# AiRyunn/BoT

Measured on NVIDIA B200. Metric: GAT layer fwd+bwd edges/sec (ogbn-proteins shape), higher is better.
Workload: dtype f32

## Files before the change

bot_b200/csrc/common.cuh:

```cuda
#pragma once

#include <atomic>
#include <cuda_runtime.h>
#include <stdint.h>
#include <stdio.h>

#include <type_traits>

#include "botgat.h"

namespace botgat {

void set_error(const char* fmt, ...);
const char* env_str(const char* name);
int64_t env_int(const char* name, int64_t dflt);
extern std::atomic<long long> g_launches;
#define BG_LAUNCHED(n) (::botgat::g_launches.fetch_add(n, std::memory_order_relaxed))

#define BG_CHECK(expr)                                                                  \
  do {                                                                                  \
    cudaError_t _e = (expr);                                                            \
    if (_e != cudaSuccess) {                                                            \
      ::botgat::set_error("%s:%d: %s -> %s", __FILE__, __LINE__, #expr, cudaGetErrorString(_e)); \
      return -2;                                                                        \
    }                                                                                   \
  } while (0)

#define BG_REQUIRE(cond, ...)            \
  do {                                   \
    if (!(cond)) {                       \
      ::botgat::set_error(__VA_ARGS__);  \
      return -1;                         \
    }                                    \
  } while (0)

struct DeviceGuard {
  int prev = -1;
  explicit DeviceGuard(int dev) {
    cudaGetDevice(&prev);
    if (dev != prev) cudaSetDevice(dev);
  }
  ~DeviceGuard() {
    int cur;
    cudaGetDevice(&cur);
    if (cur != prev && prev >= 0) cudaSetDevice(prev);
  }
};

template <typename K>
static inline int resident_grid(K kernel, int block_threads, int64_t blocks_of_work) {
  int dev = 0, sms = 148, per_sm = 1;
  cudaGetDevice(&dev);
  cudaDeviceGetAttribute(&sms, cudaDevAttrMultiProcessorCount, dev);
  if (cudaOccupancyMaxActiveBlocksPerMultiprocessor(&per_sm, kernel, block_threads, 0) != cudaSuccess || per_sm < 1) per_sm = 1;
  const int64_t resident = (int64_t)sms * per_sm;
  return (int)(blocks_of_work < 1 ? 1 : (blocks_of_work < resident ? blocks_of_work : resident));
}

}

struct botgat_graph {
  int device = 0;
  int sm_count = 148;
  int64_t n_src = 0, n_dst = 0, n_edges = 0;
  int64_t max_in_deg = 0, max_out_deg = 0;
  int has_zero_in_degree = 0;
  int32_t *in_indptr = nullptr, *in_indices = nullptr, *in_eid = nullptr;
  int32_t *out_indptr = nullptr, *out_indices = nullptr, *out_eid = nullptr;
  int32_t *in_deg = nullptr, *out_deg = nullptr;
  int in_eid_identity = 0;
  int32_t* out_tile_order = nullptr;
  int tiles_s = 1, tiles_d = 1;
  struct SegTable {
    int n_items = 0;
    int n_slots = 0;
    int n_split = 0;
    int32_t *row = nullptr, *beg = nullptr, *end = nullptr, *slot = nullptr;
    int32_t *split_rows = nullptr, *split_first = nullptr;
  } seg_in, seg_out;
};

namespace botgat {

#ifndef BG_WPB
#define BG_WPB 4
#endif
constexpr int kWarpsPerBlock = BG_WPB;
constexpr unsigned kFull = 0xffffffffu;

__device__ __forceinline__ float leaky_relu(float z, float slope) {
  return z > 0.f ? z : (z == -INFINITY ? -INFINITY : z * slope);
}

__device__ __forceinline__ float warp_max(float v) {
#pragma unroll
  for (int o = 16; o > 0; o >>= 1) v = fmaxf(v, __shfl_xor_sync(kFull, v, o));
  return v;
}
__device__ __forceinline__ float warp_sum(float v) {
#pragma unroll
  for (int o = 16; o > 0; o >>= 1) v += __shfl_xor_sync(kFull, v, o);
  return v;
}

__device__ __forceinline__ uint32_t philox_u32(uint64_t seed, uint32_t eid, uint32_t head) {
  uint32_t c0 = eid, c1 = head >> 2, c2 = 0x9E3779B9u, c3 = 0xBB67AE85u;
  uint32_t k0 = (uint32_t)seed, k1 = (uint32_t)(seed >> 32);
#pragma unroll
  for (int r = 0; r < 10; ++r) {
    uint32_t hi0 = __umulhi(0xD2511F53u, c0), lo0 = 0xD2511F53u * c0;
    uint32_t hi1 = __umulhi(0xCD9E8D57u, c2), lo1 = 0xCD9E8D57u * c2;
    uint32_t n0 = hi1 ^ c1 ^ k0, n1 = lo1, n2 = hi0 ^ c3 ^ k1, n3 = lo0;
    c0 = n0; c1 = n1; c2 = n2; c3 = n3;
    k0 += 0x9E3779B9u; k1 += 0xBB67AE85u;
  }
  uint32_t sel = head & 3u;
  return sel == 0 ? c0 : sel == 1 ? c1 : sel == 2 ? c2 : c3;
}
__device__ __forceinline__ float philox_dropout_mul(uint64_t seed, uint32_t eid, uint32_t head, float p, float inv_keep) {
  float u = (float)(philox_u32(seed, eid, head) >> 8) * (1.0f / 16777216.0f);
  return u >= p ? inv_keep : 0.f;
}

template <int VW> struct Vec;
// ... 119 lines not shown
```

bot_b200/csrc/edge_ops.cu:

```cuda
#include <cub/cub.cuh>
#include <thrust/iterator/counting_iterator.h>
#include <thrust/iterator/transform_iterator.h>

#include "common.cuh"

namespace botgat {

static int env_pf() {
  return (int)env_int("BOTGAT_PF", 0);
}

template <int PF> __device__ __forceinline__ float4 ld_rec4(const float* p) {
  float4 r;
  if constexpr (PF == 64)
    asm("ld.global.nc.L2::64B.v4.f32 {%0,%1,%2,%3}, [%4];" : "=f"(r.x), "=f"(r.y), "=f"(r.z), "=f"(r.w) : "l"(p));
  else if constexpr (PF == 128)
    asm("ld.global.nc.L2::128B.v4.f32 {%0,%1,%2,%3}, [%4];" : "=f"(r.x), "=f"(r.y), "=f"(r.z), "=f"(r.w) : "l"(p));
  else if constexpr (PF == 256)
    asm("ld.global.nc.L2::256B.v4.f32 {%0,%1,%2,%3}, [%4];" : "=f"(r.x), "=f"(r.y), "=f"(r.z), "=f"(r.w) : "l"(p));
  else
    r = __ldg(reinterpret_cast<const float4*>(p));
  return r;
}
template <int PF> __device__ __forceinline__ float2 ld_rec2(const float* p) {
// ... 9 lines not shown
  if constexpr (PF == 64) asm("ld.global.nc.L2::64B.f32 %0, [%1];" : "=f"(r) : "l"(p));
  else if constexpr (PF == 128) asm("ld.global.nc.L2::128B.f32 %0, [%1];" : "=f"(r) : "l"(p));
  else if constexpr (PF == 256) asm("ld.global.nc.L2::256B.f32 %0, [%1];" : "=f"(r) : "l"(p));
  else r = __ldg(p);
  return r;
}

constexpr int kHMax = 8;

template <int VEC, int PF> __device__ __forceinline__ void load_record(const float* rec, int H, float (&v)[kHMax]) {
  if constexpr (VEC == 4) {
#pragma unroll
    for (int q = 0; q < kHMax / 4; ++q) {
      if (q * 4 < H) {
        const float4 t = ld_rec4<PF>(rec + q * 4);
        v[q * 4] = t.x; v[q * 4 + 1] = t.y; v[q * 4 + 2] = t.z; v[q * 4 + 3] = t.w;
      }
    }
  } else if constexpr (VEC == 2) {
#pragma unroll
    for (int q = 0; q < kHMax / 2; ++q) {
      if (q * 2 < H) {
        const float2 t = ld_rec2<PF>(rec + q * 2);
        v[q * 2] = t.x; v[q * 2 + 1] = t.y;
      }
    }
  } else {
#pragma unroll
    for (int q = 0; q < kHMax; ++q)
      if (q < H) v[q] = ld_rec1<PF>(rec + q);
  }
}
template <int VEC> __device__ __forceinline__ void store_record(float* rec, int H, const float (&v)[kHMax]) {
  if constexpr (VEC == 4) {
#pragma unroll
    for (int q = 0; q < kHMax / 4; ++q)
      if (q * 4 < H) *reinterpret_cast<float4*>(rec + q * 4) = make_float4(v[q * 4], v[q * 4 + 1], v[q * 4 + 2], v[q * 4 + 3]);
  } else if constexpr (VEC == 2) {
#pragma unroll
    for (int q = 0; q < kHMax / 2; ++q)
      if (q * 2 < H) *reinterpret_cast<float2*>(rec + q * 2) = make_float2(v[q * 2], v[q * 2 + 1]);
  } else {
#pragma unroll
    for (int q = 0; q < kHMax; ++q)
      if (q < H) rec[q] = v[q];
  }
}

static int record_vec(const void* p, int64_t ld, int H) {
  auto fits = [&](int w) { return ld % w == 0 && ((uintptr_t)p % (4 * w)) == 0 && ((H + w - 1) / w) * w <= ld; };
  return fits(4) ? 4 : (fits(2) ? 2 : 1);
}

__global__ void k_pack_keep(int64_t n_edges, const uint8_t* __restrict__ keep, uint32_t* __restrict__ bits) {
  const int64_t n_round = (n_edges + 31) & ~(int64_t)31;
  for (int64_t e = blockIdx.x * (int64_t)blockDim.x + threadIdx.x; e < n_round; e += (int64_t)gridDim.x * blockDim.x) {
    const unsigned b = __ballot_sync(0xffffffffu, e < n_edges && __ldg(keep + e) != 0);
    if ((threadIdx.x & 31) == 0) bits[e >> 5] = b;
  }
}

struct KeptMap {
  const uint32_t* bits;
  const int32_t* base;
  __device__ __forceinline__ int64_t rank(int64_t x) const {
    return __ldg(base + (x >> 5)) + __popc(__ldg(bits + (x >> 5)) & ((1u << (x & 31)) - 1u));
  }
  __device__ __forceinline__ bool kept(int64_t p) const { return (__ldg(bits + (p >> 5)) >> (p & 31)) & 1u; }
};

template <int VEC, int PF>
__global__ void k_edge_stage(int64_t n_edges, int h0, int Hn, const int32_t* __restrict__ eid,
                             const int32_t* __restrict__ order,
                             const float* __restrict__ src, int64_t ld, const uint8_t* __restrict__ keep,
                             const uint32_t* __restrict__ keep_bits, float* __restrict__ dst,
                             const KeptMap km, const int32_t* __restrict__ indices,
                             int32_t* __restrict__ sub_indices, int32_t* __restrict__ sub_eid) {
  for (int64_t t = blockIdx.x * (int64_t)blockDim.x + threadIdx.x; t < n_edges; t += (int64_t)gridDim.x * blockDim.x) {
    const int64_t p = order ? __ldg(order + t) : t;
    int64_t q = p;
    if (km.bits) {
      if (!km.kept(p)) continue;
      q = km.rank(p);
    }
    const int64_t e = __ldg(eid + p);
    float v[kHMax];
#pragma unroll
    for (int c = 0; c < kHMax; ++c) v[c] = 0.f;
    if (src) load_record<VEC, PF>(src + e * ld + h0, Hn, v);
    const bool dropped = keep_bits ? !((__ldg(keep_bits + (e >> 5)) >> (e & 31)) & 1u) : (keep && !__ldg(keep + e));
#pragma unroll
    for (int c = 0; c < kHMax; ++c)
      if (c < Hn) dst[(int64_t)(h0 + c) * n_edges + q] = dropped ? -INFINITY : v[c];
    if (sub_indices) {
      sub_indices[q] = __ldg(indices + p);
      if (sub_eid) sub_eid[q] = (int32_t)e;
    }
  }
}

template <int VEC>
__global__ void k_edge_unstage(int64_t n_edges, int h0, int Hn, int Hw, const int32_t* __restrict__ eid,
                               const int32_t* __restrict__ order, const KeptMap km,
                               const float* __restrict__ gz, float* __restrict__ dst, int64_t ld) {
  for (int64_t t = blockIdx.x * (int64_t)blockDim.x + threadIdx.x; t < n_edges; t += (int64_t)gridDim.x * blockDim.x) {
    const int64_t p = order ? __ldg(order + t) : t;
    const int64_t e = __ldg(eid + p);
    int64_t q = p;
    bool kept = true;
    if (km.bits) {
      kept = km.kept(p);
      q = km.rank(p);
    }
    float v[kHMax];
#pragma unroll
    for (int c = 0; c < kHMax; ++c) v[c] = (c < Hn && kept) ? __ldg(gz + (int64_t)(h0 + c) * n_edges + q) : 0.f;
    store_record<VEC>(dst + e * ld + h0, Hw, v);
  }
}

__global__ void k_kept_bits(int64_t n_edges, int64_t n_words, const int32_t* __restrict__ eid, const uint8_t* __restrict__ keep,
                            const uint32_t* __restrict__ keep_bits, uint32_t* __restrict__ bits) {
  for (int64_t p = blockIdx.x * (int64_t)blockDim.x + threadIdx.x; p < n_words * 32; p += (int64_t)gridDim.x * blockDim.x) {
    bool k = false;
    if (p < n_edges) {
      const int64_t e = eid ? __ldg(eid + p) : p;
      k = keep_bits ? ((__ldg(keep_bits + (e >> 5)) >> (e & 31)) & 1u) : __ldg(keep + e) != 0;
    }
    const unsigned b = __ballot_sync(0xffffffffu, k);
    if ((threadIdx.x & 31) == 0) bits[p >> 5] = b;
  }
}

struct WordCount {
  const uint32_t* bits;
  __device__ int operator()(int64_t w) const { return __popc(__ldg(bits + w)); }
};

__global__ void k_subset_bounds(int n_rows, const int32_t* __restrict__ indptr, int n_seg, const int32_t* __restrict__ seg_beg,
                                const int32_t* __restrict__ seg_end, const KeptMap km,
                                int32_t* __restrict__ sub_indptr, int32_t* __restrict__ sub_beg, int32_t* __restrict__ sub_end) {
  const int n = max(n_rows + 1, n_seg);
  for (int i = blockIdx.x * blockDim.x + threadIdx.x; i < n; i += gridDim.x * blockDim.x) {
    if (i <= n_rows) sub_indptr[i] = (int32_t)km.rank(__ldg(indptr + i));
    if (i < n_seg) {
      sub_beg[i] = (int32_t)km.rank(__ldg(seg_beg + i));
      sub_end[i] = (int32_t)km.rank(__ldg(seg_end + i));
    }
  }
}

template <int VEC, int PF>
__global__ void __launch_bounds__(256)
k_edge_reduce_dst(int n_items, int H, int h0, int Hn, const int32_t* __restrict__ indptr, const int32_t* __restrict__ eid,
                  const int32_t* __restrict__ seg_row, const int32_t* __restrict__ seg_beg,
                  const int32_t* __restrict__ seg_end, const int32_t* __restrict__ seg_slot,
                  const float* __restrict__ grad_ee, int64_t ld, float* __restrict__ grad_er, float* __restrict__ scratch) {
  const int warp = threadIdx.x >> 5, lane = threadIdx.x & 31;
  const int item = blockIdx.x * 8 + warp;
  if (item >= n_items) return;
  const int v = seg_row ? seg_row[item] : item;
  const int beg = seg_row ? seg_beg[item] : indptr[v], end = seg_row ? seg_end[item] : indptr[v + 1];
  const int slot = seg_row ? seg_slot[item] : -1;
  float s[kHMax];
#pragma unroll
  for (int q = 0; q < kHMax; ++q) s[q] = 0.f;
  for (int pos = beg + lane; pos < end; pos += 32) {
    float r[kHMax];
#pragma unroll
    for (int q = 0; q < kHMax; ++q) r[q] = 0.f;
    load_record<VEC, PF>(grad_ee + (int64_t)__ldg(eid + pos) * ld + h0, Hn, r);
#pragma unroll
    for (int q = 0; q < kHMax; ++q) s[q] += r[q];
  }
#pragma unroll
  for (int q = 0; q < kHMax; ++q) {
    if (q < Hn) {
      const float t = warp_sum(s[q]);
      if (lane == 0) {
        if (slot >= 0) scratch[(int64_t)slot * H + h0 + q] = t;
        else grad_er[(int64_t)v * H + h0 + q] = t;
      }
    }
  }
}

__global__ void k_edge_reduce_combine(int n_split, int H, const int32_t* __restrict__ split_rows,
                                      const int32_t* __restrict__ split_first, const float* __restrict__ scratch,
                                      float* __restrict__ grad_er) {
  const int t = blockIdx.x * blockDim.x + threadIdx.x;
  if (t >= n_split * H) return;
  const int i = t / H, h = t - i * H;
  float a = 0.f;
  for (int s = split_first[i]; s < split_first[i + 1]; ++s) a += scratch[(int64_t)s * H + h];
  grad_er[(int64_t)split_rows[i] * H + h] = a;
}

static inline int grid_for(int64_t n, int block = 256) {
  int64_t b = (n + block - 1) / block;
  return (int)std::max<int64_t>(1, std::min<int64_t>(b, 148 * 32));
}

#define BG_PF_SWITCH(CALL)                        \
  switch (pf) {                                   \
    case 64: { constexpr int PF = 64; CALL; break; }   \
    case 128: { constexpr int PF = 128; CALL; break; } \
    case 256: { constexpr int PF = 256; CALL; break; } \
    default: { constexpr int PF = 0; CALL; break; }    \
  }

struct KeepBits {
  uint32_t* p = nullptr;
  cudaStream_t st = nullptr;
  ~KeepBits() { if (p) cudaFreeAsync(p, st); }
};
static int pack_keep_bits(const botgat_graph* g, const int32_t* eid, const uint8_t* keep, bool with_records, cudaStream_t st,
                          KeepBits* kb) {
  const bool coalesced = eid == g->in_eid && g->in_eid_identity;
  if (!keep || !with_records || g->n_edges < (1 << 20) || coalesced) return 0;
  kb->st = st;
  BG_CHECK(cudaMallocAsync(&kb->p, sizeof(uint32_t) * (size_t)((g->n_edges + 31) / 32), st));
  k_pack_keep<<<grid_for(g->n_edges), 256, 0, st>>>(g->n_edges, keep, kb->p);
  BG_LAUNCHED(1);
  return 0;
}

static int build_subset(const botgat_graph* g, int order, const uint8_t* keep, const uint32_t* keep_bits,
                        botgat_edge_subset* s, cudaStream_t st) {
  const bool in = order == BOTGAT_ORDER_IN;
  const int32_t* eid = in ? g->in_eid : g->out_eid;
  const botgat_graph::SegTable& seg = in ? g->seg_in : g->seg_out;
  const int n_rows = (int)(in ? g->n_dst : g->n_src);
  const int n_seg = seg.n_items;
  const int64_t n_words = g->n_edges / 32 + 1;
  k_kept_bits<<<grid_for(n_words * 32), 256, 0, st>>>(g->n_edges, n_words, in && g->in_eid_identity ? nullptr : eid, keep,
                                                      keep_bits, s->kept);
  BG_LAUNCHED(1);
  auto counts = thrust::make_transform_iterator(thrust::counting_iterator<int64_t>(0), WordCount{s->kept});
  size_t tb = 0;
  BG_CHECK(cub::DeviceScan::ExclusiveSum(nullptr, tb, counts, s->base, (int)n_words, st));
  void* tmp = nullptr;
  BG_CHECK(cudaMallocAsync(&tmp, tb, st));
  const cudaError_t scan = cub::DeviceScan::ExclusiveSum(tmp, tb, counts, s->base, (int)n_words, st);
  BG_LAUNCHED(1);
  BG_CHECK(cudaFreeAsync(tmp, st));
  BG_CHECK(scan);
  const KeptMap km{s->kept, s->base};
  k_subset_bounds<<<grid_for(std::max(n_rows + 1, n_seg)), 256, 0, st>>>(n_rows, in ? g->in_indptr : g->out_indptr, n_seg,
                                                                        seg.beg, seg.end, km, s->indptr, s->seg_beg,
                                                                        s->seg_end);
  BG_LAUNCHED(1);
  BG_CHECK(cudaGetLastError());
  return 0;
}

static int stage_one(const botgat_graph* g, const int32_t* eid, const int32_t* order, int H, const float* src, int64_t ld,
                     const uint8_t* keep, float* dst, const botgat_edge_subset* sub, const int32_t* indices,
                     cudaStream_t st) {
  const int pf = env_pf();
  KeepBits kb;
  if (int rc = pack_keep_bits(g, eid, keep, src != nullptr, st, &kb)) return rc;
  const uint32_t* keep_bits = kb.p;
  const KeptMap km{sub ? sub->kept : nullptr, sub ? sub->base : nullptr};
  for (int h0 = 0; h0 < H; h0 += kHMax) {
    const int Hn = std::min(kHMax, H - h0);
    const int vec = src ? record_vec(src + h0, ld, Hn) : 1;
    int32_t* sub_indices = sub && indices && h0 == 0 ? sub->indices : nullptr;
    int32_t* sub_eid = sub_indices ? sub->eid : nullptr;
    const int grid = order ? (int)((g->n_edges + 255) / 256) : grid_for(g->n_edges);
#define BG_ST(VEC) BG_PF_SWITCH((k_edge_stage<VEC, PF><<<grid, 256, 0, st>>>(g->n_edges, h0, Hn, eid, order, src, ld, keep, keep_bits, dst, km, indices, sub_indices, sub_eid)))
    if (vec == 4) { BG_ST(4) } else if (vec == 2) { BG_ST(2) } else { BG_ST(1) }
#undef BG_ST
    BG_LAUNCHED(1);
    BG_CHECK(cudaGetLastError());
  }
  return 0;
}

}

using namespace botgat;

extern "C" int botgat_edge_stage(const botgat_graph* g, int order, int32_t H, const float* ee, int64_t ld_ee,
                                 const uint8_t* keep, const float* attn_mul, int64_t ld_am, float* eb, float* am,
                                 botgat_edge_subset* subset, void* stream) {
  BG_REQUIRE(g && H > 0, "edge_stage: bad arguments");
  BG_REQUIRE(order == BOTGAT_ORDER_IN || order == BOTGAT_ORDER_OUT, "edge_stage: bad order %d", order);
  BG_REQUIRE((eb != nullptr) == (ee != nullptr || keep != nullptr), "edge_stage: eb must be given iff ee or keep is");
  BG_REQUIRE((am != nullptr) == (attn_mul != nullptr), "edge_stage: am must be given iff attn_mul is");
  BG_REQUIRE(!ee || ld_ee >= H, "edge_stage: ld_ee < H");
  BG_REQUIRE(!attn_mul || ld_am >= H, "edge_stage: ld_am < H");
  BG_REQUIRE(!subset || keep, "edge_stage: the kept-edge subset needs keep");
  const bool split = (order == BOTGAT_ORDER_IN ? g->seg_in : g->seg_out).n_items > 0;
  BG_REQUIRE(!subset || (subset->kept && subset->base && subset->indptr && subset->indices &&
                         (!split || (subset->seg_beg && subset->seg_end))),
             "edge_stage: subset needs kept, base, indptr, indices and, for a CSR with split rows, seg_beg / seg_end");
  DeviceGuard guard(g->device);
  cudaStream_t st = (cudaStream_t)stream;
  if (g->n_edges == 0) {
    if (subset)
      BG_CHECK(cudaMemsetAsync(subset->indptr, 0, sizeof(int32_t) * (size_t)((order == BOTGAT_ORDER_IN ? g->n_dst : g->n_src) + 1), st));
    return 0;
  }
  if (!eb && !am) return 0;
  const int32_t* eid = order == BOTGAT_ORDER_IN ? g->in_eid : g->out_eid;
  const int32_t* visit = order == BOTGAT_ORDER_OUT ? g->out_tile_order : nullptr;
  if (subset) {
    KeepBits kb;
    int rc = pack_keep_bits(g, eid, keep, ee != nullptr, st, &kb);
    if (!rc) rc = build_subset(g, order, keep, kb.p, subset, st);
    if (rc) return rc;
  }
  const int32_t* indices = order == BOTGAT_ORDER_IN ? g->in_indices : g->out_indices;
  if (eb) {
    int rc = stage_one(g, eid, visit, ee ? H : 1, ee, ld_ee, subset ? nullptr : keep, eb, subset, indices, st);
    if (rc) return rc;
  }
  if (am) {
    int rc = stage_one(g, eid, visit, H, attn_mul, ld_am, nullptr, am, subset, nullptr, st);
    if (rc) return rc;
  }
  return 0;
}

extern "C" int botgat_edge_unstage(const botgat_graph* g, int order, int32_t H, const float* gz, float* grad_ee,
                                   int64_t ld_gee, const botgat_edge_subset* subset, void* stream) {
  BG_REQUIRE(g && H > 0, "edge_unstage: bad arguments");
  BG_REQUIRE(order == BOTGAT_ORDER_IN || order == BOTGAT_ORDER_OUT, "edge_unstage: bad order %d", order);
  if (g->n_edges == 0) return 0;
  BG_REQUIRE(gz && grad_ee, "edge_unstage: null gz/grad_ee");
  BG_REQUIRE(ld_gee >= H, "edge_unstage: ld_gee < H");
  BG_REQUIRE(!subset || (subset->kept && subset->base), "edge_unstage: subset without kept / base");
  DeviceGuard guard(g->device);
  cudaStream_t st = (cudaStream_t)stream;
  const int32_t* eid = order == BOTGAT_ORDER_IN ? g->in_eid : g->out_eid;
  const int32_t* visit = order == BOTGAT_ORDER_OUT ? g->out_tile_order : nullptr;
  const KeptMap km{subset ? subset->kept : nullptr, subset ? subset->base : nullptr};
  for (int h0 = 0; h0 < ld_gee; h0 += kHMax) {
    const int Hn = std::max(0, std::min(kHMax, H - h0));
    const int Hw = (int)std::min<int64_t>(kHMax, ld_gee - h0);
    const int vec = record_vec(grad_ee + h0, ld_gee, Hw);
    const int grid = visit ? (int)((g->n_edges + 255) / 256) : grid_for(g->n_edges);
    if (vec == 4) k_edge_unstage<4><<<grid, 256, 0, st>>>(g->n_edges, h0, Hn, Hw, eid, visit, km, gz, grad_ee, ld_gee);
    else if (vec == 2) k_edge_unstage<2><<<grid, 256, 0, st>>>(g->n_edges, h0, Hn, Hw, eid, visit, km, gz, grad_ee, ld_gee);
    else k_edge_unstage<1><<<grid, 256, 0, st>>>(g->n_edges, h0, Hn, Hw, eid, visit, km, gz, grad_ee, ld_gee);
    BG_LAUNCHED(1);
    BG_CHECK(cudaGetLastError());
  }
  return 0;
}

extern "C" int botgat_edge_reduce_dst(const botgat_graph* g, int32_t H, const float* grad_ee, int64_t ld_gee,
                                      float* grad_er, float* scratch, void* stream) {
  BG_REQUIRE(g && H > 0 && grad_er, "edge_reduce_dst: bad arguments");
  BG_REQUIRE(grad_ee || g->n_edges == 0, "edge_reduce_dst: null grad_ee");
  BG_REQUIRE(ld_gee >= H || g->n_edges == 0, "edge_reduce_dst: ld_gee < H");
  if (g->n_dst == 0) return 0;
  DeviceGuard guard(g->device);
  cudaStream_t st = (cudaStream_t)stream;
  const int pf = env_pf();
  const botgat_graph::SegTable& seg = g->seg_in;
  const bool split = seg.n_items > 0;
  BG_REQUIRE(!split || seg.n_slots == 0 || scratch, "edge_reduce_dst: this graph has split rows; scratch (n_slots_in*H floats) is required");
  const int n_items = split ? seg.n_items : (int)g->n_dst;
  const int32_t *sr = split ? seg.row : nullptr, *sb = seg.beg, *se = seg.end, *ss = seg.slot;
  const int grid = (n_items + 7) / 8;
  for (int h0 = 0; h0 < H; h0 += kHMax) {
    const int Hn = std::min(kHMax, H - h0);
    const int vec = g->n_edges ? record_vec(grad_ee + h0, ld_gee, Hn) : 1;
#define BG_RD(VEC) BG_PF_SWITCH((k_edge_reduce_dst<VEC, PF><<<grid, 256, 0, st>>>(n_items, H, h0, Hn, g->in_indptr, g->in_eid, sr, sb, se, ss, grad_ee, ld_gee, grad_er, scratch)))
    if (vec == 4) { BG_RD(4) } else if (vec == 2) { BG_RD(2) } else { BG_RD(1) }
#undef BG_RD
    BG_LAUNCHED(1);
    BG_CHECK(cudaGetLastError());
  }
  if (split && seg.n_split > 0) {
    const int n = seg.n_split * H;
    k_edge_reduce_combine<<<(n + 255) / 256, 256, 0, st>>>(seg.n_split, H, seg.split_rows, seg.split_first, scratch, grad_er);
    BG_LAUNCHED(1);
    BG_CHECK(cudaGetLastError());
  }
  return 0;
}
```

bot_b200/csrc/graph.cu:

```cuda
#include <cub/cub.cuh>

#include <atomic>
#include <cstdarg>
#include <cstring>

#include "common.cuh"

namespace botgat {

static thread_local char g_err[512] = "";
std::atomic<long long> g_launches{0};

void set_error(const char* fmt, ...) {
  va_list ap;
  va_start(ap, fmt);
  vsnprintf(g_err, sizeof(g_err), fmt, ap);
  va_end(ap);
}

__global__ void k_narrow_and_check(int64_t n, const int64_t* __restrict__ a, int64_t bound, int32_t* __restrict__ out,
                                   int32_t* __restrict__ iota, int* __restrict__ bad) {
  for (int64_t i = blockIdx.x * (int64_t)blockDim.x + threadIdx.x; i < n; i += (int64_t)gridDim.x * blockDim.x) {
    const int64_t v = a[i];
    const bool oob = v < 0 || v >= bound;
// ... 2 lines not shown
    if (iota) iota[i] = (int32_t)i;
  }
}

__global__ void k_histogram(int64_t n, const int32_t* __restrict__ keys, int32_t* __restrict__ counts) {
  for (int64_t i = blockIdx.x * (int64_t)blockDim.x + threadIdx.x; i < n; i += (int64_t)gridDim.x * blockDim.x)
    atomicAdd(counts + keys[i], 1);
}

__global__ void k_gather_i32(int64_t n, const int32_t* __restrict__ table, const int32_t* __restrict__ idx,
                             int32_t* __restrict__ out) {
  for (int64_t i = blockIdx.x * (int64_t)blockDim.x + threadIdx.x; i < n; i += (int64_t)gridDim.x * blockDim.x)
    out[i] = table[idx[i]];
}

__global__ void k_deg_stats(int64_t n, const int32_t* __restrict__ deg, int* __restrict__ stats) {
  int mx = 0, zeros = 0;
  for (int64_t i = blockIdx.x * (int64_t)blockDim.x + threadIdx.x; i < n; i += (int64_t)gridDim.x * blockDim.x) {
    const int d = deg[i];
    mx = max(mx, d);
    zeros += d == 0;
  }
  for (int o = 16; o > 0; o >>= 1) {
    mx = max(mx, __shfl_xor_sync(kFull, mx, o));
    zeros += __shfl_xor_sync(kFull, zeros, o);
  }
  if ((threadIdx.x & 31) == 0) {
    atomicMax(stats, mx);
    atomicAdd(stats + 1, zeros);
  }
}

static inline int grid_for(int64_t n, int block = 256) {
  int64_t b = (n + block - 1) / block;
  return (int)std::max<int64_t>(1, std::min<int64_t>(b, 148 * 32));
}

__global__ void k_check_identity(int64_t n, const int32_t* __restrict__ eid, int* __restrict__ flag) {
  for (int64_t i = blockIdx.x * (int64_t)blockDim.x + threadIdx.x; i < n; i += (int64_t)gridDim.x * blockDim.x)
    if (eid[i] != (int32_t)i) *flag = 1;
}

__global__ void k_tile_keys(int n_src, const int32_t* __restrict__ indptr, const int32_t* __restrict__ indices,
                            int rows_per_s, int rows_per_d, int tiles_d, int32_t* __restrict__ keys,
                            int32_t* __restrict__ iota) {
  const int warp = (blockIdx.x * blockDim.x + threadIdx.x) >> 5, lane = threadIdx.x & 31;
  const int nwarps = (gridDim.x * blockDim.x) >> 5;
  for (int r = warp; r < n_src; r += nwarps) {
    const int ts = r / rows_per_s;
    for (int p = indptr[r] + lane; p < indptr[r + 1]; p += 32) {
      keys[p] = ts * tiles_d + indices[p] / rows_per_d;
      iota[p] = p;
    }
  }
}

static int bits_for(int64_t n) {
  int b = 1;
  while ((1ll << b) < n) ++b;
  return b;
}

static int build_csr(int64_t n_rows, int64_t n_edges, const int32_t* key, const int32_t* other, const int32_t* iota,
                     int32_t* key_sorted_tmp, int32_t* indptr, int32_t* indices, int32_t* eid, int32_t* deg,
                     cudaStream_t st) {
  if (n_edges > 0) {
    size_t tmp_bytes = 0;
    BG_CHECK(cub::DeviceRadixSort::SortPairs(nullptr, tmp_bytes, key, key_sorted_tmp, iota, eid, (int)n_edges, 0,
                                             bits_for(n_rows), st));
    void* tmp = nullptr;
    BG_CHECK(cudaMallocAsync(&tmp, tmp_bytes, st));
    BG_CHECK(cub::DeviceRadixSort::SortPairs(tmp, tmp_bytes, key, key_sorted_tmp, iota, eid, (int)n_edges, 0,
                                             bits_for(n_rows), st)); BG_LAUNCHED(1);
    BG_CHECK(cudaFreeAsync(tmp, st));
    k_gather_i32<<<grid_for(n_edges), 256, 0, st>>>(n_edges, other, eid, indices); BG_LAUNCHED(1);
    BG_CHECK(cudaGetLastError());
  }
  BG_CHECK(cudaMemsetAsync(deg, 0, sizeof(int32_t) * (n_rows + 1), st));
  if (n_edges > 0) {
    k_histogram<<<grid_for(n_edges), 256, 0, st>>>(n_edges, key, deg); BG_LAUNCHED(1);
    BG_CHECK(cudaGetLastError());
  }
  {
    size_t tmp_bytes = 0;
    BG_CHECK(cub::DeviceScan::ExclusiveSum(nullptr, tmp_bytes, deg, indptr, (int)(n_rows + 1), st));
    void* tmp = nullptr;
    BG_CHECK(cudaMallocAsync(&tmp, tmp_bytes, st));
    BG_CHECK(cub::DeviceScan::ExclusiveSum(tmp, tmp_bytes, deg, indptr, (int)(n_rows + 1), st)); BG_LAUNCHED(1);
    BG_CHECK(cudaFreeAsync(tmp, st));
  }
  return 0;
}

}

using namespace botgat;

extern "C" int botgat_abi_version(void) { return BOTGAT_ABI_VERSION; }
extern "C" const char* botgat_last_error(void) { return g_err; }
extern "C" int64_t botgat_launch_count(void) { return (int64_t)g_launches.load(); }

static void configure_pool(int device) {
  static std::atomic<unsigned> done{0};
  const unsigned bit = 1u << (device & 31);
  if (done.fetch_or(bit) & bit) return;
  cudaMemPool_t pool;
  if (cudaDeviceGetDefaultMemPool(&pool, device) != cudaSuccess) return;
  uint64_t thr = 0;
  if (cudaMemPoolGetAttribute(pool, cudaMemPoolAttrReleaseThreshold, &thr) == cudaSuccess && thr == 0) {
    thr = 2ull << 30;
    cudaMemPoolSetAttribute(pool, cudaMemPoolAttrReleaseThreshold, &thr);
  }
}

static void destroy_impl(botgat_graph* g, bool async, cudaStream_t st) {
  if (!g) return;
  DeviceGuard guard(g->device);
  void* ptrs[] = {g->in_indptr, g->in_indices, g->in_eid, g->out_indptr, g->out_indices, g->out_eid, g->in_deg, g->out_deg};
  for (void* q : ptrs) {
    if (!q) continue;
    if (!async || cudaFreeAsync(q, st) != cudaSuccess) { cudaGetLastError(); cudaFree(q); }
  }
  if (g->out_tile_order && (!async || cudaFreeAsync(g->out_tile_order, st) != cudaSuccess)) { cudaGetLastError(); cudaFree(g->out_tile_order); }
  free_segments(&g->seg_in, async, st); free_segments(&g->seg_out, async, st);
  delete g;
}

extern "C" void botgat_graph_destroy(botgat_graph* g) { destroy_impl(g, false, nullptr); }
extern "C" void botgat_graph_destroy_async(botgat_graph* g, void* stream) { destroy_impl(g, true, (cudaStream_t)stream); }

extern "C" int botgat_graph_create(int64_t n_src, int64_t n_dst, int64_t n_edges, const int64_t* src,
                                   const int64_t* dst, int device, void* stream, botgat_graph** out) {
  BG_REQUIRE(out, "graph_create: null out");
  *out = nullptr;
  BG_REQUIRE(n_src >= 0 && n_dst >= 0 && n_edges >= 0, "graph_create: negative size");
  BG_REQUIRE(n_edges < (1ll << 31) - 1 && n_src < (1ll << 31) - 1 && n_dst < (1ll << 31) - 1,
             "graph_create: sizes must be < 2^31-1 (int32 structure arrays)");
  BG_REQUIRE(n_edges == 0 || (src && dst), "graph_create: null src/dst");
  DeviceGuard guard(device);
  cudaStream_t st = (cudaStream_t)stream;

  botgat_graph* g = new botgat_graph();
  g->device = device; g->n_src = n_src; g->n_dst = n_dst; g->n_edges = n_edges;
  cudaDeviceGetAttribute(&g->sm_count, cudaDevAttrMultiProcessorCount, device);
  struct Cleanup {
    botgat_graph*& g;
    bool armed = true;
    ~Cleanup() { if (armed) { botgat_graph_destroy(g); } }
  } cleanup{g};

  configure_pool(device);
  const size_t eb = sizeof(int32_t) * (size_t)std::max<int64_t>(n_edges, 1);
  BG_CHECK(cudaMallocAsync(&g->in_indptr, sizeof(int32_t) * (n_dst + 1), st));
  BG_CHECK(cudaMallocAsync(&g->out_indptr, sizeof(int32_t) * (n_src + 1), st));
  BG_CHECK(cudaMallocAsync(&g->in_indices, eb, st)); BG_CHECK(cudaMallocAsync(&g->in_eid, eb, st));
  BG_CHECK(cudaMallocAsync(&g->out_indices, eb, st)); BG_CHECK(cudaMallocAsync(&g->out_eid, eb, st));
  BG_CHECK(cudaMallocAsync(&g->in_deg, sizeof(int32_t) * (n_dst + 1), st));
  BG_CHECK(cudaMallocAsync(&g->out_deg, sizeof(int32_t) * (n_src + 1), st));

  int32_t *src32 = nullptr, *dst32 = nullptr, *iota = nullptr, *ktmp = nullptr;
  int* flags = nullptr;
  BG_CHECK(cudaMallocAsync(&src32, eb, st)); BG_CHECK(cudaMallocAsync(&dst32, eb, st));
  BG_CHECK(cudaMallocAsync(&iota, eb, st)); BG_CHECK(cudaMallocAsync(&ktmp, eb, st));
  BG_CHECK(cudaMallocAsync(&flags, sizeof(int) * 6, st));
  BG_CHECK(cudaMemsetAsync(flags, 0, sizeof(int) * 6, st));
  if (n_edges > 0) {
    k_narrow_and_check<<<grid_for(n_edges), 256, 0, st>>>(n_edges, src, n_src, src32, iota, flags); BG_LAUNCHED(1);
    k_narrow_and_check<<<grid_for(n_edges), 256, 0, st>>>(n_edges, dst, n_dst, dst32, nullptr, flags); BG_LAUNCHED(1);
    BG_CHECK(cudaGetLastError());
  }
  int rc = build_csr(n_dst, n_edges, dst32, src32, iota, ktmp, g->in_indptr, g->in_indices, g->in_eid, g->in_deg, st);
  if (rc) return rc;
  rc = build_csr(n_src, n_edges, src32, dst32, iota, ktmp, g->out_indptr, g->out_indices, g->out_eid, g->out_deg, st);
  if (rc) return rc;
  if (n_dst > 0) k_deg_stats<<<grid_for(n_dst), 256, 0, st>>>(n_dst, g->in_deg, flags + 1); BG_LAUNCHED(1);
  if (n_src > 0) k_deg_stats<<<grid_for(n_src), 256, 0, st>>>(n_src, g->out_deg, flags + 3); BG_LAUNCHED(1);
  if (n_edges > 0) k_check_identity<<<grid_for(n_edges), 256, 0, st>>>(n_edges, g->in_eid, flags + 5); BG_LAUNCHED(1);
  BG_CHECK(cudaGetLastError());
  int h[6];
  BG_CHECK(cudaMemcpyAsync(h, flags, sizeof(h), cudaMemcpyDeviceToHost, st));
  BG_CHECK(cudaFreeAsync(src32, st)); BG_CHECK(cudaFreeAsync(dst32, st));
  BG_CHECK(cudaFreeAsync(flags, st));
  BG_CHECK(cudaStreamSynchronize(st));
  if (h[0] != 0) { cudaFreeAsync(iota, st); cudaFreeAsync(ktmp, st); }
  BG_REQUIRE(h[0] == 0, "graph_create: node id out of range [0,n_src) / [0,n_dst)");
  g->max_in_deg = h[1]; g->has_zero_in_degree = h[2] > 0; g->max_out_deg = h[3];
  g->in_eid_identity = h[5] == 0;
  {
    int ts = 1, td = 1;
    const char* force = env_str("BOTGAT_TILES");
    if (force) {
      if (sscanf(force, "%d,%d", &ts, &td) != 2) ts = td = 1;
    } else if (g->in_eid_identity && n_edges >= (1 << 22) && n_src > 0 && n_dst > 0) {
      const double avg_in = (double)n_edges / n_dst, avg_out = (double)n_edges / n_src;
      const int cap_s = std::max(1, (int)(avg_in / 16)), cap_d = std::max(1, (int)(avg_out / 16));
      const double need = (double)n_edges * 32.0 / ((double)env_int("BOTGAT_TILE_MB", 20) * (1 << 20));
      int want = 1;
      while ((double)want * want < need) ++want;
      ts = std::min(want, cap_s); td = std::min(want, cap_d);
      while ((double)ts * td < need && ts < cap_s) ++ts;
      while ((double)ts * td < need && td < cap_d) ++td;
      if ((double)ts * td < need * 0.5) ts = td = 1;
    }
    ts = std::max(1, std::min(ts, 64)); td = std::max(1, std::min(td, 64));
    if (ts * td > 1 && n_edges > 0 && n_src > 0 && n_dst > 0) {
      const int rows_per_s = (int)((n_src + ts - 1) / ts), rows_per_d = (int)((n_dst + td - 1) / td);
      BG_CHECK(cudaMallocAsync(&g->out_tile_order, eb, st));
      k_tile_keys<<<grid_for(n_src * 32), 256, 0, st>>>((int)n_src, g->out_indptr, g->out_indices, rows_per_s, rows_per_d,
                                                       td, ktmp, iota); BG_LAUNCHED(1);
      int32_t* ksorted = nullptr;
      BG_CHECK(cudaMallocAsync(&ksorted, eb, st));
      size_t tmp_bytes = 0;
      const int kbits = bits_for((int64_t)ts * td);
      BG_CHECK(cub::DeviceRadixSort::SortPairs(nullptr, tmp_bytes, ktmp, ksorted, iota, g->out_tile_order, (int)n_edges, 0, kbits, st));
      void* tmp = nullptr;
      BG_CHECK(cudaMallocAsync(&tmp, tmp_bytes, st));
      BG_CHECK(cub::DeviceRadixSort::SortPairs(tmp, tmp_bytes, ktmp, ksorted, iota, g->out_tile_order, (int)n_edges, 0, kbits, st)); BG_LAUNCHED(1);
      BG_CHECK(cudaFreeAsync(tmp, st)); BG_CHECK(cudaFreeAsync(ksorted, st));
      g->tiles_s = ts; g->tiles_d = td;
    }
  }
  BG_CHECK(cudaFreeAsync(iota, st)); BG_CHECK(cudaFreeAsync(ktmp, st));
  rc = build_segments((int)n_dst, g->in_indptr, g->in_deg, g->max_in_deg, &g->seg_in, st);
  if (rc) return rc;
  rc = build_segments((int)n_src, g->out_indptr, g->out_deg, g->max_out_deg, &g->seg_out, st);
  if (rc) return rc;
  cleanup.armed = false;
  *out = g;
  return 0;
}

extern "C" int botgat_graph_get(const botgat_graph* g, int which, void** dev_ptr, int64_t* len) {
  BG_REQUIRE(g && dev_ptr && len, "graph_get: null argument");
  switch (which) {
    case BOTGAT_IN_INDPTR: *dev_ptr = g->in_indptr; *len = g->n_dst + 1; break;
    case BOTGAT_IN_INDICES: *dev_ptr = g->in_indices; *len = g->n_edges; break;
    case BOTGAT_IN_EID: *dev_ptr = g->in_eid; *len = g->n_edges; break;
    case BOTGAT_OUT_INDPTR: *dev_ptr = g->out_indptr; *len = g->n_src + 1; break;
    case BOTGAT_OUT_INDICES: *dev_ptr = g->out_indices; *len = g->n_edges; break;
    case BOTGAT_OUT_EID: *dev_ptr = g->out_eid; *len = g->n_edges; break;
    case BOTGAT_IN_DEG: *dev_ptr = g->in_deg; *len = g->n_dst; break;
    case BOTGAT_OUT_DEG: *dev_ptr = g->out_deg; *len = g->n_src; break;
    default: set_error("graph_get: unknown array %d", which); return -1;
  }
  return 0;
}

extern "C" int botgat_graph_get_info(const botgat_graph* g, botgat_graph_info* info) {
  BG_REQUIRE(g && info, "graph_get_info: null argument");
  info->n_src = g->n_src; info->n_dst = g->n_dst; info->n_edges = g->n_edges;
  info->max_in_deg = g->max_in_deg; info->max_out_deg = g->max_out_deg;
  info->has_zero_in_degree = g->has_zero_in_degree; info->device = g->device;
  info->n_slots_in = g->seg_in.n_slots; info->n_slots_out = g->seg_out.n_slots;
  info->in_eid_identity = g->in_eid_identity; info->tiles_src = g->tiles_s; info->tiles_dst = g->tiles_d;
  info->n_seg_in = g->seg_in.n_items; info->n_seg_out = g->seg_out.n_items; info->reserved_ = 0;
  return 0;
}

namespace botgat {

__global__ void k_pack_bidirected(int64_t n, const int64_t* __restrict__ src, const int64_t* __restrict__ dst,
                                  int64_t n_nodes, uint64_t* __restrict__ keys, int* __restrict__ bad) {
  for (int64_t i = blockIdx.x * (int64_t)blockDim.x + threadIdx.x; i < n; i += (int64_t)gridDim.x * blockDim.x) {
    const int64_t s = src[i], d = dst[i];
    if (s < 0 || s >= n_nodes || d < 0 || d >= n_nodes) *bad = 1;
    keys[i] = (uint64_t)s * (uint64_t)n_nodes + (uint64_t)d;
    keys[n + i] = (uint64_t)d * (uint64_t)n_nodes + (uint64_t)s;
  }
}
__global__ void k_unpack(int64_t n, const uint64_t* __restrict__ keys, int64_t n_nodes, int64_t* __restrict__ src,
                         int64_t* __restrict__ dst) {
// ... 246 lines not shown
```

Before: 2.888 billion.

## Precompute tiled visit (pos,eid) pairs and batch edge stage/unstage per thread

Replaces the out-order tile permutation with a precomputed int2 array of (position, edge id), so staging kernels read both in one load rather than chasing order and then eid. New visit kernels handle several edges per thread and issue all loads before the stores to raise memory-level parallelism. The kept-bits kernel now builds one word per thread with vectorized byte loads in place of warp ballots, and the identity eid is skipped in the in-order paths. The cost is twice the memory for the visit table and more registers per thread.

```diff
diff --git a/bot_b200/csrc/common.cuh b/bot_b200/csrc/common.cuh
--- a/bot_b200/csrc/common.cuh
+++ b/bot_b200/csrc/common.cuh
@@ -69,7 +69,7 @@
   int32_t *out_indptr = nullptr, *out_indices = nullptr, *out_eid = nullptr;
   int32_t *in_deg = nullptr, *out_deg = nullptr;
   int in_eid_identity = 0;
-  int32_t* out_tile_order = nullptr;
+  int2* out_visit = nullptr;
   int tiles_s = 1, tiles_d = 1;
   struct SegTable {
     int n_items = 0;
diff --git a/bot_b200/csrc/edge_ops.cu b/bot_b200/csrc/edge_ops.cu
--- a/bot_b200/csrc/edge_ops.cu
+++ b/bot_b200/csrc/edge_ops.cu
@@ -85,12 +85,48 @@
   return fits(4) ? 4 : (fits(2) ? 2 : 1);
 }
 
-__global__ void k_pack_keep(int64_t n_edges, const uint8_t* __restrict__ keep, uint32_t* __restrict__ bits) {
-  const int64_t n_round = (n_edges + 31) & ~(int64_t)31;
-  for (int64_t e = blockIdx.x * (int64_t)blockDim.x + threadIdx.x; e < n_round; e += (int64_t)gridDim.x * blockDim.x) {
-    const unsigned b = __ballot_sync(0xffffffffu, e < n_edges && __ldg(keep + e) != 0);
-    if ((threadIdx.x & 31) == 0) bits[e >> 5] = b;
-  }
+__device__ __forceinline__ uint32_t nonzero_bytes(uint4 x) {
+  uint32_t b = 0;
+  const uint32_t w[4] = {x.x, x.y, x.z, x.w};
+#pragma unroll
+  for (int i = 0; i < 16; ++i) b |= (uint32_t)(((w[i >> 2] >> (8 * (i & 3))) & 0xffu) != 0) << i;
+  return b;
+}
+
+__global__ void k_kept_bits(int64_t n_edges, int64_t n_words, const int32_t* __restrict__ eid, const uint8_t* __restrict__ keep,
+                            const uint32_t* __restrict__ keep_bits, uint32_t* __restrict__ bits) {
+  const int64_t w = blockIdx.x * (int64_t)blockDim.x + threadIdx.x;
+  if (w >= n_words) return;
+  const int64_t p0 = w * 32;
+  uint32_t b = 0;
+  if (p0 + 32 <= n_edges && !eid && !keep_bits && ((uintptr_t)keep & 15) == 0) {
+    const uint4* k4 = reinterpret_cast<const uint4*>(keep + p0);
+    b = nonzero_bytes(__ldg(k4)) | nonzero_bytes(__ldg(k4 + 1)) << 16;
+  } else if (p0 + 32 <= n_edges) {
+    int32_t e[32];
+    if (eid) {
+#pragma unroll
+      for (int q = 0; q < 8; ++q) {
+        const int4 v = __ldg(reinterpret_cast<const int4*>(eid + p0) + q);
+        e[4 * q] = v.x; e[4 * q + 1] = v.y; e[4 * q + 2] = v.z; e[4 * q + 3] = v.w;
+      }
+    } else {
+#pragma unroll
+      for (int i = 0; i < 32; ++i) e[i] = (int32_t)(p0 + i);
+    }
+#pragma unroll
+    for (int i = 0; i < 32; ++i) {
+      const bool k = keep_bits ? (__ldg(keep_bits + (e[i] >> 5)) >> (e[i] & 31)) & 1u : __ldg(keep + e[i]) != 0;
+      b |= (uint32_t)k << i;
+    }
+  } else {
+    for (int i = 0; i < 32 && p0 + i < n_edges; ++i) {
+      const int64_t e = eid ? __ldg(eid + p0 + i) : p0 + i;
+      const bool k = keep_bits ? (__ldg(keep_bits + (e >> 5)) >> (e & 31)) & 1u : __ldg(keep + e) != 0;
+      b |= (uint32_t)k << i;
+    }
+  }
+  bits[w] = b;
 }
 
 struct KeptMap {
@@ -104,19 +140,17 @@
 
 template <int VEC, int PF>
 __global__ void k_edge_stage(int64_t n_edges, int h0, int Hn, const int32_t* __restrict__ eid,
-                             const int32_t* __restrict__ order,
                              const float* __restrict__ src, int64_t ld, const uint8_t* __restrict__ keep,
                              const uint32_t* __restrict__ keep_bits, float* __restrict__ dst,
                              const KeptMap km, const int32_t* __restrict__ indices,
                              int32_t* __restrict__ sub_indices, int32_t* __restrict__ sub_eid) {
-  for (int64_t t = blockIdx.x * (int64_t)blockDim.x + threadIdx.x; t < n_edges; t += (int64_t)gridDim.x * blockDim.x) {
-    const int64_t p = order ? __ldg(order + t) : t;
+  for (int64_t p = blockIdx.x * (int64_t)blockDim.x + threadIdx.x; p < n_edges; p += (int64_t)gridDim.x * blockDim.x) {
     int64_t q = p;
     if (km.bits) {
       if (!km.kept(p)) continue;
       q = km.rank(p);
     }
-    const int64_t e = __ldg(eid + p);
+    const int64_t e = eid ? __ldg(eid + p) : p;
     float v[kHMax];
 #pragma unroll
     for (int c = 0; c < kHMax; ++c) v[c] = 0.f;
@@ -132,13 +166,81 @@
   }
 }
 
+#ifndef BG_VISIT_K
+#define BG_VISIT_K 4
+#endif
+constexpr int kVisitPerThread = BG_VISIT_K;
+
+template <int K>
+__device__ __forceinline__ void visit_targets(int64_t n_edges, int64_t t0, const int2* __restrict__ visit, const KeptMap& km,
+                                              int2 (&pe)[K], bool (&on)[K], int64_t (&q)[K]) {
+#pragma unroll
+  for (int i = 0; i < K; ++i) {
+    const int64_t t = t0 + i * 256;
+    pe[i] = t < n_edges ? __ldg(visit + t) : make_int2(0, 0);
+    on[i] = t < n_edges;
+  }
+  if (km.bits) {
+    uint32_t w[K];
+    int32_t b[K];
+#pragma unroll
+    for (int i = 0; i < K; ++i) {
+      w[i] = on[i] ? __ldg(km.bits + (pe[i].x >> 5)) : 0u;
+      b[i] = on[i] ? __ldg(km.base + (pe[i].x >> 5)) : 0;
+    }
+#pragma unroll
+    for (int i = 0; i < K; ++i) {
+      on[i] = on[i] && ((w[i] >> (pe[i].x & 31)) & 1u);
+      q[i] = b[i] + __popc(w[i] & ((1u << (pe[i].x & 31)) - 1u));
+    }
+  } else {
+#pragma unroll
+    for (int i = 0; i < K; ++i) q[i] = pe[i].x;
+  }
+}
+
+template <int VEC, int PF>
+__global__ void __launch_bounds__(256)
+k_edge_stage_visit(int64_t n_edges, int h0, int Hn, const int2* __restrict__ visit,
+                   const float* __restrict__ src, int64_t ld, const uint8_t* __restrict__ keep,
+                   const uint32_t* __restrict__ keep_bits, float* __restrict__ dst,
+                   const KeptMap km, const int32_t* __restrict__ indices,
+                   int32_t* __restrict__ sub_indices, int32_t* __restrict__ sub_eid) {
+  constexpr int K = kVisitPerThread;
+  int2 pe[K];
+  bool on[K];
+  int64_t q[K];
+  visit_targets<K>(n_edges, (int64_t)blockIdx.x * (256 * K) + threadIdx.x, visit, km, pe, on, q);
+  float v[K][kHMax];
+  bool dropped[K];
+  int32_t idx[K];
+#pragma unroll
+  for (int i = 0; i < K; ++i) {
+#pragma unroll
+    for (int c = 0; c < kHMax; ++c) v[i][c] = 0.f;
+    const int64_t e = pe[i].y;
+    if (on[i] && src) load_record<VEC, PF>(src + e * ld + h0, Hn, v[i]);
+    dropped[i] = on[i] && (keep_bits ? !((__ldg(keep_bits + (e >> 5)) >> (e & 31)) & 1u) : (keep && !__ldg(keep + e)));
+    idx[i] = on[i] && sub_indices ? __ldg(indices + pe[i].x) : 0;
+  }
+#pragma unroll
+  for (int i = 0; i < K; ++i) {
+    if (!on[i]) continue;
+#pragma unroll
+    for (int c = 0; c < kHMax; ++c)
+      if (c < Hn) dst[(int64_t)(h0 + c) * n_edges + q[i]] = dropped[i] ? -INFINITY : v[i][c];
+    if (sub_indices) {
+      sub_indices[q[i]] = idx[i];
+      if (sub_eid) sub_eid[q[i]] = pe[i].y;
+    }
+  }
+}
+
 template <int VEC>
-__global__ void k_edge_unstage(int64_t n_edges, int h0, int Hn, int Hw, const int32_t* __restrict__ eid,
-                               const int32_t* __restrict__ order, const KeptMap km,
+__global__ void k_edge_unstage(int64_t n_edges, int h0, int Hn, int Hw, const int32_t* __restrict__ eid, const KeptMap km,
                                const float* __restrict__ gz, float* __restrict__ dst, int64_t ld) {
-  for (int64_t t = blockIdx.x * (int64_t)blockDim.x + threadIdx.x; t < n_edges; t += (int64_t)gridDim.x * blockDim.x) {
-    const int64_t p = order ? __ldg(order + t) : t;
-    const int64_t e = __ldg(eid + p);
+  for (int64_t p = blockIdx.x * (int64_t)blockDim.x + threadIdx.x; p < n_edges; p += (int64_t)gridDim.x * blockDim.x) {
+    const int64_t e = eid ? __ldg(eid + p) : p;
     int64_t q = p;
     bool kept = true;
     if (km.bits) {
@@ -152,17 +254,24 @@
   }
 }
 
-__global__ void k_kept_bits(int64_t n_edges, int64_t n_words, const int32_t* __restrict__ eid, const uint8_t* __restrict__ keep,
-                            const uint32_t* __restrict__ keep_bits, uint32_t* __restrict__ bits) {
-  for (int64_t p = blockIdx.x * (int64_t)blockDim.x + threadIdx.x; p < n_words * 32; p += (int64_t)gridDim.x * blockDim.x) {
-    bool k = false;
-    if (p < n_edges) {
-      const int64_t e = eid ? __ldg(eid + p) : p;
-      k = keep_bits ? ((__ldg(keep_bits + (e >> 5)) >> (e & 31)) & 1u) : __ldg(keep + e) != 0;
-    }
-    const unsigned b = __ballot_sync(0xffffffffu, k);
-    if ((threadIdx.x & 31) == 0) bits[p >> 5] = b;
-  }
+template <int VEC>
+__global__ void __launch_bounds__(256)
+k_edge_unstage_visit(int64_t n_edges, int h0, int Hn, int Hw, const int2* __restrict__ visit, const KeptMap km,
+                     const float* __restrict__ gz, float* __restrict__ dst, int64_t ld) {
+  constexpr int K = kVisitPerThread;
+  int2 pe[K];
+  bool on[K];
+  int64_t q[K];
+  const int64_t t0 = (int64_t)blockIdx.x * (256 * K) + threadIdx.x;
+  visit_targets<K>(n_edges, t0, visit, km, pe, on, q);
+  float v[K][kHMax];
+#pragma unroll
+  for (int i = 0; i < K; ++i)
+#pragma unroll
+    for (int c = 0; c < kHMax; ++c) v[i][c] = (c < Hn && on[i]) ? __ldg(gz + (int64_t)(h0 + c) * n_edges + q[i]) : 0.f;
+#pragma unroll
+  for (int i = 0; i < K; ++i)
+    if (t0 + i * 256 < n_edges) store_record<VEC>(dst + (int64_t)pe[i].y * ld + h0, Hw, v[i]);
 }
 
 struct WordCount {
@@ -202,7 +311,7 @@
     float r[kHMax];
 #pragma unroll
     for (int q = 0; q < kHMax; ++q) r[q] = 0.f;
-    load_record<VEC, PF>(grad_ee + (int64_t)__ldg(eid + pos) * ld + h0, Hn, r);
+    load_record<VEC, PF>(grad_ee + (eid ? (int64_t)__ldg(eid + pos) : (int64_t)pos) * ld + h0, Hn, r);
 #pragma unroll
     for (int q = 0; q < kHMax; ++q) s[q] += r[q];
   }
@@ -242,6 +351,17 @@
     default: { constexpr int PF = 0; CALL; break; }    \
   }
 
+struct Walk {
+  const int32_t* eid;
+  const int2* visit;
+};
+static Walk walk_of(const botgat_graph* g, int order) {
+  if (order == BOTGAT_ORDER_IN) return {g->in_eid_identity ? nullptr : g->in_eid, nullptr};
+  return {g->out_eid, g->out_visit};
+}
+
+static inline int visit_grid(int64_t n) { return (int)((n + 256 * kVisitPerThread - 1) / (256 * kVisitPerThread)); }
+
 struct KeepBits {
   uint32_t* p = nullptr;
   cudaStream_t st = nullptr;
@@ -249,11 +369,12 @@
 };
 static int pack_keep_bits(const botgat_graph* g, const int32_t* eid, const uint8_t* keep, bool with_records, cudaStream_t st,
                           KeepBits* kb) {
-  const bool coalesced = eid == g->in_eid && g->in_eid_identity;
+  const bool coalesced = eid == nullptr;
   if (!keep || !with_records || g->n_edges < (1 << 20) || coalesced) return 0;
   kb->st = st;
-  BG_CHECK(cudaMallocAsync(&kb->p, sizeof(uint32_t) * (size_t)((g->n_edges + 31) / 32), st));
-  k_pack_keep<<<grid_for(g->n_edges), 256, 0, st>>>(g->n_edges, keep, kb->p);
+  const int64_t n_words = (g->n_edges + 31) / 32;
+  BG_CHECK(cudaMallocAsync(&kb->p, sizeof(uint32_t) * (size_t)n_words, st));
+  k_kept_bits<<<(int)((n_words + 255) / 256), 256, 0, st>>>(g->n_edges, n_words, nullptr, keep, nullptr, kb->p);
   BG_LAUNCHED(1);
   return 0;
 }
@@ -261,13 +382,11 @@
 static int build_subset(const botgat_graph* g, int order, const uint8_t* keep, const uint32_t* keep_bits,
                         botgat_edge_subset* s, cudaStream_t st) {
   const bool in = order == BOTGAT_ORDER_IN;
-  const int32_t* eid = in ? g->in_eid : g->out_eid;
   const botgat_graph::SegTable& seg = in ? g->seg_in : g->seg_out;
   const int n_rows = (int)(in ? g->n_dst : g->n_src);
   const int n_seg = seg.n_items;
   const int64_t n_words = g->n_edges / 32 + 1;
-  k_kept_bits<<<grid_for(n_words * 32), 256, 0, st>>>(g->n_edges, n_words, in && g->in_eid_identity ? nullptr : eid, keep,
-                                                      keep_bits, s->kept);
+  k_kept_bits<<<(int)((n_words + 255) / 256), 256, 0, st>>>(g->n_edges, n_words, walk_of(g, order).eid, keep, keep_bits, s->kept);
   BG_LAUNCHED(1);
   auto counts = thrust::make_transform_iterator(thrust::counting_iterator<int64_t>(0), WordCount{s->kept});
   size_t tb = 0;
@@ -287,12 +406,11 @@
   return 0;
 }
 
-static int stage_one(const botgat_graph* g, const int32_t* eid, const int32_t* order, int H, const float* src, int64_t ld,
-                     const uint8_t* keep, float* dst, const botgat_edge_subset* sub, const int32_t* indices,
-                     cudaStream_t st) {
+static int stage_one(const botgat_graph* g, const Walk& w, int H, const float* src, int64_t ld, const uint8_t* keep,
+                     float* dst, const botgat_edge_subset* sub, const int32_t* indices, cudaStream_t st) {
   const int pf = env_pf();
   KeepBits kb;
-  if (int rc = pack_keep_bits(g, eid, keep, src != nullptr, st, &kb)) return rc;
+  if (int rc = pack_keep_bits(g, w.eid, keep, src != nullptr, st, &kb)) return rc;
   const uint32_t* keep_bits = kb.p;
   const KeptMap km{sub ? sub->kept : nullptr, sub ? sub->base : nullptr};
   for (int h0 = 0; h0 < H; h0 += kHMax) {
@@ -300,10 +418,15 @@
     const int vec = src ? record_vec(src + h0, ld, Hn) : 1;
     int32_t* sub_indices = sub && indices && h0 == 0 ? sub->indices : nullptr;
     int32_t* sub_eid = sub_indices ? sub->eid : nullptr;
-    const int grid = order ? (int)((g->n_edges + 255) / 256) : grid_for(g->n_edges);
-#define BG_ST(VEC) BG_PF_SWITCH((k_edge_stage<VEC, PF><<<grid, 256, 0, st>>>(g->n_edges, h0, Hn, eid, order, src, ld, keep, keep_bits, dst, km, indices, sub_indices, sub_eid)))
-    if (vec == 4) { BG_ST(4) } else if (vec == 2) { BG_ST(2) } else { BG_ST(1) }
+    if (w.visit) {
+#define BG_ST(VEC) BG_PF_SWITCH((k_edge_stage_visit<VEC, PF><<<visit_grid(g->n_edges), 256, 0, st>>>(g->n_edges, h0, Hn, w.visit, src, ld, keep, keep_bits, dst, km, indices, sub_indices, sub_eid)))
+      if (vec == 4) { BG_ST(4) } else if (vec == 2) { BG_ST(2) } else { BG_ST(1) }
 #undef BG_ST
+    } else {
+#define BG_ST(VEC) BG_PF_SWITCH((k_edge_stage<VEC, PF><<<grid_for(g->n_edges), 256, 0, st>>>(g->n_edges, h0, Hn, w.eid, src, ld, keep, keep_bits, dst, km, indices, sub_indices, sub_eid)))
+      if (vec == 4) { BG_ST(4) } else if (vec == 2) { BG_ST(2) } else { BG_ST(1) }
+#undef BG_ST
+    }
     BG_LAUNCHED(1);
     BG_CHECK(cudaGetLastError());
   }
@@ -336,21 +459,20 @@
     return 0;
   }
   if (!eb && !am) return 0;
-  const int32_t* eid = order == BOTGAT_ORDER_IN ? g->in_eid : g->out_eid;
-  const int32_t* visit = order == BOTGAT_ORDER_OUT ? g->out_tile_order : nullptr;
+  const Walk w = walk_of(g, order);
   if (subset) {
     KeepBits kb;
-    int rc = pack_keep_bits(g, eid, keep, ee != nullptr, st, &kb);
+    int rc = pack_keep_bits(g, w.eid, keep, ee != nullptr, st, &kb);
     if (!rc) rc = build_subset(g, order, keep, kb.p, subset, st);
     if (rc) return rc;
   }
   const int32_t* indices = order == BOTGAT_ORDER_IN ? g->in_indices : g->out_indices;
   if (eb) {
-    int rc = stage_one(g, eid, visit, ee ? H : 1, ee, ld_ee, subset ? nullptr : keep, eb, subset, indices, st);
+    int rc = stage_one(g, w, ee ? H : 1, ee, ld_ee, subset ? nullptr : keep, eb, subset, indices, st);
     if (rc) return rc;
   }
   if (am) {
-    int rc = stage_one(g, eid, visit, H, attn_mul, ld_am, nullptr, am, subset, nullptr, st);
+    int rc = stage_one(g, w, H, attn_mul, ld_am, nullptr, am, subset, nullptr, st);
     if (rc) return rc;
   }
   return 0;
@@ -366,17 +488,17 @@
   BG_REQUIRE(!subset || (subset->kept && subset->base), "edge_unstage: subset without kept / base");
   DeviceGuard guard(g->device);
   cudaStream_t st = (cudaStream_t)stream;
-  const int32_t* eid = order == BOTGAT_ORDER_IN ? g->in_eid : g->out_eid;
-  const int32_t* visit = order == BOTGAT_ORDER_OUT ? g->out_tile_order : nullptr;
+  const Walk w = walk_of(g, order);
   const KeptMap km{subset ? subset->kept : nullptr, subset ? subset->base : nullptr};
   for (int h0 = 0; h0 < ld_gee; h0 += kHMax) {
     const int Hn = std::max(0, std::min(kHMax, H - h0));
     const int Hw = (int)std::min<int64_t>(kHMax, ld_gee - h0);
     const int vec = record_vec(grad_ee + h0, ld_gee, Hw);
-    const int grid = visit ? (int)((g->n_edges + 255) / 256) : grid_for(g->n_edges);
-    if (vec == 4) k_edge_unstage<4><<<grid, 256, 0, st>>>(g->n_edges, h0, Hn, Hw, eid, visit, km, gz, grad_ee, ld_gee);
-    else if (vec == 2) k_edge_unstage<2><<<grid, 256, 0, st>>>(g->n_edges, h0, Hn, Hw, eid, visit, km, gz, grad_ee, ld_gee);
-    else k_edge_unstage<1><<<grid, 256, 0, st>>>(g->n_edges, h0, Hn, Hw, eid, visit, km, gz, grad_ee, ld_gee);
+#define BG_US(VEC)                                                                                                        \
+  if (w.visit) k_edge_unstage_visit<VEC><<<visit_grid(g->n_edges), 256, 0, st>>>(g->n_edges, h0, Hn, Hw, w.visit, km, gz, grad_ee, ld_gee); \
+  else k_edge_unstage<VEC><<<grid_for(g->n_edges), 256, 0, st>>>(g->n_edges, h0, Hn, Hw, w.eid, km, gz, grad_ee, ld_gee);
+    if (vec == 4) { BG_US(4) } else if (vec == 2) { BG_US(2) } else { BG_US(1) }
+#undef BG_US
     BG_LAUNCHED(1);
     BG_CHECK(cudaGetLastError());
   }
@@ -401,7 +523,7 @@
   for (int h0 = 0; h0 < H; h0 += kHMax) {
     const int Hn = std::min(kHMax, H - h0);
     const int vec = g->n_edges ? record_vec(grad_ee + h0, ld_gee, Hn) : 1;
-#define BG_RD(VEC) BG_PF_SWITCH((k_edge_reduce_dst<VEC, PF><<<grid, 256, 0, st>>>(n_items, H, h0, Hn, g->in_indptr, g->in_eid, sr, sb, se, ss, grad_ee, ld_gee, grad_er, scratch)))
+#define BG_RD(VEC) BG_PF_SWITCH((k_edge_reduce_dst<VEC, PF><<<grid, 256, 0, st>>>(n_items, H, h0, Hn, g->in_indptr, walk_of(g, BOTGAT_ORDER_IN).eid, sr, sb, se, ss, grad_ee, ld_gee, grad_er, scratch)))
     if (vec == 4) { BG_RD(4) } else if (vec == 2) { BG_RD(2) } else { BG_RD(1) }
 #undef BG_RD
     BG_LAUNCHED(1);
diff --git a/bot_b200/csrc/graph.cu b/bot_b200/csrc/graph.cu
--- a/bot_b200/csrc/graph.cu
+++ b/bot_b200/csrc/graph.cu
@@ -78,6 +78,14 @@
       keys[p] = ts * tiles_d + indices[p] / rows_per_d;
       iota[p] = p;
     }
+  }
+}
+
+__global__ void k_visit_pairs(int64_t n, const int32_t* __restrict__ pos, const int32_t* __restrict__ eid,
+                              int2* __restrict__ visit) {
+  for (int64_t t = blockIdx.x * (int64_t)blockDim.x + threadIdx.x; t < n; t += (int64_t)gridDim.x * blockDim.x) {
+    const int32_t p = pos[t];
+    visit[t] = make_int2(p, eid[p]);
   }
 }
 
@@ -147,7 +155,7 @@
     if (!q) continue;
     if (!async || cudaFreeAsync(q, st) != cudaSuccess) { cudaGetLastError(); cudaFree(q); }
   }
-  if (g->out_tile_order && (!async || cudaFreeAsync(g->out_tile_order, st) != cudaSuccess)) { cudaGetLastError(); cudaFree(g->out_tile_order); }
+  if (g->out_visit && (!async || cudaFreeAsync(g->out_visit, st) != cudaSuccess)) { cudaGetLastError(); cudaFree(g->out_visit); }
   free_segments(&g->seg_in, async, st); free_segments(&g->seg_out, async, st);
   delete g;
 }
@@ -231,18 +239,21 @@
     ts = std::max(1, std::min(ts, 64)); td = std::max(1, std::min(td, 64));
     if (ts * td > 1 && n_edges > 0 && n_src > 0 && n_dst > 0) {
       const int rows_per_s = (int)((n_src + ts - 1) / ts), rows_per_d = (int)((n_dst + td - 1) / td);
-      BG_CHECK(cudaMallocAsync(&g->out_tile_order, eb, st));
+      BG_CHECK(cudaMallocAsync(&g->out_visit, sizeof(int2) * (size_t)n_edges, st));
       k_tile_keys<<<grid_for(n_src * 32), 256, 0, st>>>((int)n_src, g->out_indptr, g->out_indices, rows_per_s, rows_per_d,
                                                        td, ktmp, iota); BG_LAUNCHED(1);
-      int32_t* ksorted = nullptr;
-      BG_CHECK(cudaMallocAsync(&ksorted, eb, st));
+      int32_t *ksorted = nullptr, *pos = nullptr;
+      BG_CHECK(cudaMallocAsync(&ksorted, eb, st)); BG_CHECK(cudaMallocAsync(&pos, eb, st));
       size_t tmp_bytes = 0;
       const int kbits = bits_for((int64_t)ts * td);
-      BG_CHECK(cub::DeviceRadixSort::SortPairs(nullptr, tmp_bytes, ktmp, ksorted, iota, g->out_tile_order, (int)n_edges, 0, kbits, st));
+      BG_CHECK(cub::DeviceRadixSort::SortPairs(nullptr, tmp_bytes, ktmp, ksorted, iota, pos, (int)n_edges, 0, kbits, st));
       void* tmp = nullptr;
       BG_CHECK(cudaMallocAsync(&tmp, tmp_bytes, st));
-      BG_CHECK(cub::DeviceRadixSort::SortPairs(tmp, tmp_bytes, ktmp, ksorted, iota, g->out_tile_order, (int)n_edges, 0, kbits, st)); BG_LAUNCHED(1);
+      BG_CHECK(cub::DeviceRadixSort::SortPairs(tmp, tmp_bytes, ktmp, ksorted, iota, pos, (int)n_edges, 0, kbits, st)); BG_LAUNCHED(1);
       BG_CHECK(cudaFreeAsync(tmp, st)); BG_CHECK(cudaFreeAsync(ksorted, st));
+      k_visit_pairs<<<grid_for(n_edges), 256, 0, st>>>(n_edges, pos, g->out_eid, g->out_visit); BG_LAUNCHED(1);
+      BG_CHECK(cudaGetLastError());
+      BG_CHECK(cudaFreeAsync(pos, st));
       g->tiles_s = ts; g->tiles_d = td;
     }
   }
```

Result: faster. 2.945 billion, median of 6 (+2.0%).
